# zhangyi-3/UCDIR

Measured on AMD Instinct MI355X. Metric: restored images/sec at 50-step p_sample_loop, 256x256 SID, higher is better.
Workload: dtype bf16

## Files before the change

### ucdir_amd/csrc/engine.hip

```cpp
#include <hip/hip_runtime.h>

#include <cmath>
#include <cstdio>
#include <cstring>
#include <map>
#include <mutex>
#include <set>
#include <array>
#include <atomic>
#include <memory>
#include <string>
#include <vector>

#include "../../include/ucdir_hip.h"
#include "cgemm.hip.h"
#include "conv_halo.hip.h"
#include "akgm_halo.hip.h"
#include "akgm_pre.hip.h"
#include "akgm_ws.hip.h"
#include "akgm_ws32.hip.h"
#include "akgm_ws64.hip.h"
#include "conv_ws.hip.h"
#include "conv_sk.hip.h"
#include "conv_ws128.hip.h"
// ... 714 lines not shown
        nblk *= p.usplit;
    }
    p.own_tc = !env().no_owntc && w.Tbb != nullptr;
    p.Tbb = w.Tbb; p.Tgt = w.Tg;

    AkgmKind kind = pre ? AkgmKind::PRE : (!env().no_attlds && (w.cg == 16 || w.cg == 32)) ? AkgmKind::HALO_ATTLDS : AkgmKind::HALO_STAGE;
    const bool use_ws = !env().no_ws;
    if (pre && use_ws && w.C == 64 && y.H % 16 == 0 && y.W % 16 == 0 && p.th == 16 && p.tw == 16 &&
        (g_persist_grid > 0 || (long long)y.B * p.tiles_x * p.tiles_y >= 4LL * num_cus()))
        kind = AkgmKind::WS;
    if (use_ws && !env().no_ws16 && w.Apre != nullptr && w.cg == 16 && w.C == 128 && y.H % 16 == 0 && y.W % 16 == 0 &&
        (g_persist_grid > 0 || (long long)y.B * (y.H / 16) * (y.W / 16) * 2 >= 4LL * num_cus()))
        kind = AkgmKind::WS16;
    int th32 = 0;
    for (int cand : {32, 24, 16, 8}) if (y.H % cand == 0) { th32 = cand; break; }
    const bool wsb_all = g_wsb > 0;
    const int nb32 = w.C / 32;
    if (use_ws && !env().no_ws32 && w.Aws32 != nullptr && (w.cg == 32 || (wsb_all && (w.cg == 16 || w.cg == 8))) && w.C == 8 * w.cg && th32 > 0 && y.W % 8 == 0 &&
        (g_persist_grid > 0 || (long long)y.B * (y.H / th32) * (y.W / 8) * nb32 >= 4LL * num_cus()))
        kind = AkgmKind::WS32;
    int tps64 = 0, grid64 = 0, hpos64 = 0;
    if (use_ws && !env().no_ws64 && w.Aws64 != nullptr && w.cg == 64 && w.C == 512 && y.H >= 2 && (y.H + 2) * (y.W + 2) < 32768) {
        const int nrole = 128 / AkWs64::NW;
        grid64 = num_cus() / nrole * nrole; if (grid64 < nrole) grid64 = nrole;
        const int span = (y.H - 1) * (y.W + 2) + y.W, nslots = grid64 / nrole;
        for (int cand : {4, 2}) {
            const int hpos = 32 * cand + 2 * (y.W + 2) + 2;
            if (hpos > AkWs64::HPOS) continue;
            const int tps = (span + 32 * cand - 1) / (32 * cand);
            const bool enough = cand == 4 ? (long long)y.B * tps >= 4LL * nslots : 2LL * y.B * span >= 3LL * nslots * hpos;
            if (g_persist_grid > 0 || enough) {
                kind = cand == 4 ? AkgmKind::WS64_4 : AkgmKind::WS64_2;
                tps64 = tps; hpos64 = hpos;
                break;
            }
        }
    }

    void (*kernel)(AkgmHP) = akgm_halo_stage_kernel;
    int key = KEY_AKGM_HALO, grid = nblk, threads = HC_THREADS, lds = AH_LDS;
    switch (kind) {
        case AkgmKind::WS64_4: case AkgmKind::WS64_2:
            p.A = w.Aws64; p.th = kind == AkgmKind::WS64_4 ? 4 : 2; p.tw = AkWs64::HBYTES(hpos64); p.tiles_x = tps64; p.tiles_y = 1;
            kernel = kind == AkgmKind::WS64_4 ? akgm_ws64_kernel<4, 8, true> : akgm_ws64_kernel<2, 8, true>;
            key = KEY_AKGM_WS64; grid = grid64; threads = 512; lds = AkWs64::lds(hpos64);
            break;
        case AkgmKind::WS32: {
            p.A = w.Aws32; p.th = th32; p.tw = 8; p.tiles_x = y.W / 8; p.tiles_y = y.H / th32;
            const int ntiles = y.B * p.tiles_x * p.tiles_y;
            int ncu = num_cus() / nb32 * nb32; if (ncu < nb32) ncu = nb32;
            grid = nb32 * ntiles < ncu ? nb32 * ntiles : ncu;
            kernel = w.cg == 32 ? akgm_ws32_kernel<32> : w.cg == 16 ? akgm_ws32_kernel<16> : akgm_ws32_kernel<8>;
            key = KEY_AKGM_WS32; lds = AkWs32::LDS;
            break;
        }
        case AkgmKind::WS: {
            const int ntiles = y.B * p.tiles_x * p.tiles_y, ncu = num_cus();
            grid = ntiles < ncu ? ntiles : ncu;
            kernel = akgm_ws_kernel<8>; key = KEY_AKGM_WS; lds = AkWs::LDS;
            break;
        }
        case AkgmKind::WS16: {
            p.A = w.Apre; p.th = 16; p.tw = 16; p.tiles_x = y.W / 16; p.tiles_y = y.H / 16;
            int ncu = num_cus() & ~1; if (ncu < 2) ncu = 2;
            const int ntiles = y.B * p.tiles_x * p.tiles_y;
            grid = 2 * ntiles < ncu ? 2 * ntiles : ncu;
            kernel = akgm_ws_kernel<16>; key = KEY_AKGM_WS16; lds = AkWs::LDS;
            break;
        }
        case AkgmKind::PRE: kernel = akgm_pre_kernel<8>; key = KEY_AKGM_PRE; lds = AkPre<8>::LDS; break;
        case AkgmKind::HALO_ATTLDS: kernel = akgm_halo_kernel<true>; break;
        case AkgmKind::HALO_STAGE: break;
    }
    if (!p.own_tc)
        hipLaunchKernelGGL(akgm_tc_kernel, dim3(9 * ((8 * w.C + 1023) / 1024), y.B), dim3(256), 0, st, h1.stats, inv_cnt, w.bias, w.Tb, w.Tg, 8 * w.C, tcbuf, msbuf);
    const ProfEntry e{key, 2.0 * 9 * w.C * (double)w.C * y.H * y.W * y.B, (3.0 * w.C * 2 + 32) * (double)y.H * y.W * y.B + 9.0 * w.C * w.C * 2, y.H, y.W, w.C, w.C};
    StampDump sd(st, STAMPS_256); p.dbg = sd.dbg();
    bracket(e, st, [&] { hipLaunchKernelGGL(kernel, dim3(grid), dim3(threads), lds, st, p); });
    sd.print([&](int, int n) { fprintf(stderr, "AKGM TIMING cg=%d n=%d:", w.cg, n); });
}

static void run_akgm(const AkgmW& w, const Act& h1, const float* G, const float* attw, const Act& res, Act& y,
                     float* tcbuf, hipStream_t st) {
    const int C = w.C;
    require(C == 64 || C % 128 == 0, "AKGM: channel count must be 64 or a multiple of 128");
    if (g_use_halo && (w.cg == 8 || w.cg == 16 || w.cg == 32 || w.cg == 64)) { run_akgm_halo(w, h1, G, attw, res, y, tcbuf, st); return; }
    require(w.Kpad != 640, "AKGM weights packed for the halo kernel");
    GemmP p; zero_gemm(p);
    const int TM = (C == 64) ? 64 : 128;
    p.A = w.A; p.a_ld = w.Kpad; p.a_rows = C; p.a_gstride = (long long)C * w.Kpad;
    p.B0 = h1.p; p.b0_bstride = h1.bstride(); p.ld0 = C; p.c0 = C;
    p.cols_mode = COLS_S1;
    p.H = y.H; p.W = y.W; p.Wp = y.W + 2; p.Hi = y.H; p.Wi = y.W; p.Wpi = p.Wp;
    p.p0 = p.Wp + 1; p.pn = (y.H - 1) * p.Wp + y.W;
    p.ntaps = 9; p.cg = w.cg; p.cpt = w.cg / 8; p.cpt_shift = ilog2(p.cpt);
    p.nk = w.Kpad / CG_BK;
    p.tiles = (p.pn + CG_TP - 1) / CG_TP;
    p.groups_per_wg = (C == 64) ? 8 : 1;
    p.rowtiles = (C == 64) ? 1 : 8 * (C / TM);
    p.nbatch = y.B;
    p.fold = 1; p.act = 1;
    p.stats0 = h1.stats; p.inv_count = 1.0 / ((double)C * h1.H * h1.W);
    p.bias = w.bias; p.Tb = w.Tb; p.Tg = w.Tg; p.tab_ld = 8 * C;
    p.res = res.p; p.res_bstride = res.bstride(); p.res_ld = res.C; p.res_coff = 0;
    p.out = y.p; p.out_bstride = y.bstride(); p.out_ld = C; p.nfeat = C;
    p.G = G; p.g_bstride = (long long)y.H * y.W * 8; p.attw = attw;
    p.stats_out = y.stats;
    launch_cgemm(p, TM, EPI_AKGM, st);
}

struct AttnBufs {
    bf16_t* qkv = nullptr;
    float* S = nullptr;
    bf16_t* P = nullptr;
    bf16_t* Vt = nullptr;
    int N = 0, Npad = 0, C = 0, B = 0;
    bool flash = true, half = false;
};

static std::atomic<int> g_flash{-1};
static bool flash_ok(int C) {
    const bool on = g_flash < 0 ? !env().no_flash : g_flash != 0;
    return on && C % 128 == 0 && C <= 512;
}

static void alloc_attn(DevPool& pool, AttnBufs& a, int B, int N, int C, bool half) {
    a.B = B; a.N = N; a.C = C; a.Npad = ((N + 63) / 64) * 64;
    a.half = half; a.flash = flash_ok(C);
    if (a.flash && !half && g_flash < 0 && B * ((N + FA_BQ - 1) / FA_BQ) < 32) a.flash = false;
    require(a.flash || !half, "fp16 attention operands need the flash kernel (C % 128 == 0, C <= 512)");
    a.qkv = (bf16_t*)pool.alloc((size_t)B * N * 3 * C * 2);
    if (!a.flash) {
        a.S = (float*)pool.alloc((size_t)B * N * a.Npad * 4);
        a.P = (bf16_t*)pool.alloc((size_t)B * N * a.Npad * 2);
    }
    a.Vt = (bf16_t*)pool.alloc((size_t)B * C * a.Npad * 2);
}

static std::vector<float> fold_out_into_v(const float* wqkv, const float* wout, int C) {
    std::vector<float> w(wqkv, wqkv + (size_t)3 * C * C);
    std::vector<double> row(C);
    for (int o = 0; o < C; ++o) {
        for (int i = 0; i < C; ++i) row[i] = 0.0;
        for (int m = 0; m < C; ++m) {
            const double a = wout[(size_t)o * C + m];
            const float* wv = wqkv + ((size_t)2 * C + m) * C;
            for (int i = 0; i < C; ++i) row[i] += a * (double)wv[i];
        }
        for (int i = 0; i < C; ++i) w[((size_t)2 * C + o) * C + i] = (float)row[i];
    }
    return w;
}

static void run_attention(const ConvW& wqkv, const ConvW& wout, const Act& x, Act& y, AttnBufs& a, hipStream_t st) {
    const int C = x.C, N = x.H * x.W, B = x.B, Npad = ((N + 63) / 64) * 64;
    require(C % 128 == 0, "attention: channels must be a multiple of 128");
    require((size_t)N <= (size_t)a.N && C == a.C && B <= a.B, "attention buffers too small");
    const bool qws = !env().no_qkv_ws && wqkv.Aqkv && !a.half && (C == 256 || C == 512);
    if (qws) {
        QkvP q;
        q.A = wqkv.Aqkv; q.x = x.p; q.x_bstride = x.bstride();
        q.H = x.H; q.W = x.W; q.Wp = x.W + 2; q.N = N; q.nbatch = B; q.tps = (N + 127) / 128; q.rowtiles = 3 * C / 256;
        q.stats = x.stats; q.inv_count = 1.0 / ((double)C * N);
        q.Tb = wqkv.Tb; q.Tg = wqkv.Tg;
        q.qkv = a.qkv; q.qkv_bstride = (long long)N * 3 * C; q.ld = 3 * C;
        q.vt = a.Vt; q.vt_bstride = (long long)C * Npad; q.Npad = Npad;
        const int units = q.rowtiles * B * q.tps, ncu = num_cus();
        const int grid = units < ncu ? units : ncu;
        const ProfEntry e{KEY_QKV_WS, 2.0 * 3 * C * (double)C * N * B, ((double)N * C * 2 + (double)N * 3 * C * 2) * B + 3.0 * C * C * 2, x.H, x.W, C, 3 * C};
        bracket(e, st, [&] {
            if (C == 512) hipLaunchKernelGGL(qkv_ws_kernel<512>, dim3(grid), dim3(HC_THREADS), QkvWs::LDS, st, q);
            else hipLaunchKernelGGL(qkv_ws_kernel<256>, dim3(grid), dim3(HC_THREADS), QkvWs::LDS, st, q);
        });
    } else {
    {
        GemmP p; zero_gemm(p);
        p.A = wqkv.A; p.a_ld = wqkv.Kpad; p.a_rows = wqkv.rows_pad;
        p.B0 = x.p; p.b0_bstride = x.bstride(); p.ld0 = C; p.c0 = C;
        p.cols_mode = COLS_S1; p.H = x.H; p.W = x.W; p.Wp = x.W + 2; p.Hi = x.H; p.Wi = x.W; p.Wpi = p.Wp;
        p.p0 = p.Wp + 1; p.pn = (x.H - 1) * p.Wp + x.W;
        p.ntaps = 1; p.cg = C; p.cpt = C / 8; p.nk = C / CG_BK;
        p.tiles = (p.pn + CG_TP - 1) / CG_TP; p.rowtiles = wqkv.rows_pad / 128; p.nbatch = B;
        p.fold = 1; p.stats0 = x.stats; p.inv_count = 1.0 / ((double)C * N);
        p.Tb = wqkv.Tb; p.Tg = wqkv.Tg; p.tab_ld = 3 * C; p.bias = nullptr;
        p.out = a.qkv; p.out_bstride = (long long)N * 3 * C; p.out_ld = 3 * C; p.out_compact = 1; p.nfeat = 3 * C;
        p.out_f16 = a.half ? 1 : 0;
        launch_cgemm(p, 128, EPI_STD, st);
    }
    hipLaunchKernelGGL(transpose_v_kernel, dim3((Npad + 31) / 32, C / 32, B), dim3(256), 0, st,
                       a.qkv, N, 3 * C, 2 * C, C, Npad, a.Vt);
    }
    if (a.flash) {
        FlashP f;
        f.qkv = a.qkv; f.qkv_bstride = (long long)N * 3 * C; f.ld = 3 * C;
        f.vt = a.Vt; f.vt_bstride = (long long)C * Npad; f.Npad = Npad;
        f.N = N; f.C = C; f.W = x.W;
        f.scale_log2e = 1.4426950408889634f / sqrtf((float)C);
        f.bias = wout.bias;
        f.res = x.p; f.res_bstride = x.bstride(); f.out = y.p; f.out_bstride = y.bstride();
        f.stats_out = y.stats;
        f.nq = (N + FA_BQ - 1) / FA_BQ;
        StampDump sd(st, STAMPS_256); f.dbg = sd.dbg();
        const dim3 grid((unsigned)(B * f.nq));
        const size_t lds = fa_lds_bytes(C);
        const ProfEntry e{a.half ? KEY_FLASH_F16 : KEY_FLASH, 4.0 * (double)N * N * C * B, ((double)N * 3 * C * 2 + 2.0 * N * C * 2) * B, x.H, x.W, C, C};
        bracket(e, st, [&] {
            switch (C / 128 * 2 + (a.half ? 1 : 0)) {
                case 2: hipLaunchKernelGGL((flash_attn2_kernel<1, false>), grid, dim3(FA_THREADS), lds, st, f); break;
                case 3: hipLaunchKernelGGL((flash_attn2_kernel<1, true>), grid, dim3(FA_THREADS), lds, st, f); break;
                case 4: hipLaunchKernelGGL((flash_attn2_kernel<2, false>), grid, dim3(FA_THREADS), lds, st, f); break;
                case 5: hipLaunchKernelGGL((flash_attn2_kernel<2, true>), grid, dim3(FA_THREADS), lds, st, f); break;
                case 6: hipLaunchKernelGGL((flash_attn2_kernel<3, false>), grid, dim3(FA_THREADS), lds, st, f); break;
                case 7: hipLaunchKernelGGL((flash_attn2_kernel<3, true>), grid, dim3(FA_THREADS), lds, st, f); break;
                case 8: hipLaunchKernelGGL((flash_attn2_kernel<4, false>), grid, dim3(FA_THREADS), lds, st, f); break;
                default: hipLaunchKernelGGL((flash_attn2_kernel<4, true>), grid, dim3(FA_THREADS), lds, st, f); break;
            }
        });
        sd.print([&](int, int n) { fprintf(stderr, "FLASH TIMING N=%d C=%d B=%d stamps=%d:", N, C, B, n); });
        return;
    }
    {
        GemmP p; zero_gemm(p);
        p.A = a.qkv + C; p.a_bstride = (long long)N * 3 * C; p.a_ld = 3 * C; p.a_rows = N;
        p.B0 = a.qkv; p.b0_bstride = (long long)N * 3 * C; p.ld0 = 3 * C; p.c0 = C;
        p.cols_mode = COLS_PLAIN; p.H = 1; p.W = N; p.Wp = N; p.p0 = 0; p.pn = N;
        p.ntaps = 1; p.cg = C; p.cpt = C / 8; p.nk = C / CG_BK;
        p.tiles = (N + CG_TP - 1) / CG_TP; p.rowtiles = (N + 127) / 128; p.nbatch = B;
        p.alpha = 1.0f / sqrtf((float)C);
        p.out = a.S; p.out_f32 = 1; p.out_bstride = (long long)N * Npad; p.out_ld = Npad; p.nfeat = N;
        launch_cgemm(p, 128, EPI_STD, st);
    }
    {
        const long long rows = (long long)B * N;
        const dim3 g((unsigned)((rows + 3) / 4));
        if (Npad <= 64 * 4 * 2) hipLaunchKernelGGL((softmax_kernel<2>), g, dim3(256), 0, st, a.S, a.P, rows, N, Npad);
        else if (Npad <= 64 * 4 * 6) hipLaunchKernelGGL((softmax_kernel<6>), g, dim3(256), 0, st, a.S, a.P, rows, N, Npad);
        else hipLaunchKernelGGL((softmax_kernel<0>), g, dim3(256), 0, st, a.S, a.P, rows, N, Npad);
    }
    {
        GemmP p; zero_gemm(p);
        p.A = a.Vt; p.a_bstride = (long long)C * Npad; p.a_ld = Npad; p.a_rows = C;
        p.B0 = a.P; p.b0_bstride = (long long)N * Npad; p.ld0 = Npad; p.c0 = Npad;
        p.cols_mode = COLS_PLAIN; p.H = 1; p.W = N; p.Wp = N; p.p0 = 0; p.pn = N;
        p.ntaps = 1; p.cg = Npad; p.cpt = Npad / 8; p.nk = Npad / CG_BK;
        p.tiles = (N + CG_TP - 1) / CG_TP; p.rowtiles = C / 128; p.nbatch = B;
        p.bias = wout.bias;
        p.plain_w = x.W;
        p.res = x.p; p.res_bstride = x.bstride(); p.res_ld = C;
        p.out = y.p; p.out_bstride = y.bstride(); p.out_ld = C; p.nfeat = C;
        p.stats_out = y.stats;
        launch_cgemm(p, 128, EPI_STD, st);
    }
    HIPC(hipGetLastError());
}

struct LayerDesc {
    std::string kind, name;
    int level = 0, cin = 0, cout = 0, skip_c = 0; bool attn = false, push_skip = false;
};

static std::vector<LayerDesc> build_layers(const ucdir_config& c) {
    std::vector<LayerDesc> L;
    const int inner = c.inner_channel, nm = c.n_mults;
    int pre = inner, res = c.image_size, level = 0, idx = 1;
    std::vector<int> feat{pre};
    auto in_attn = [&](int r) { for (int i = 0; i < c.n_attn_res; ++i) if (c.attn_res[i] == r) return true; return false; };
    { LayerDesc d; d.kind = "stem"; d.name = "downs.0"; d.cin = c.in_channel; d.cout = inner; d.push_skip = true; L.push_back(d); }
    for (int ind = 0; ind < nm; ++ind) {
        const bool last = ind == nm - 1, ua = in_attn(res);
        const int cm = inner * c.channel_mults[ind];
        for (int r = 0; r < c.res_blocks; ++r) {
            LayerDesc d; d.kind = "block"; d.name = "downs." + std::to_string(idx++); d.level = level;
            d.cin = pre; d.cout = cm; d.attn = ua; d.push_skip = true; L.push_back(d);
            feat.push_back(cm); pre = cm;
        }
        if (!last) {
            LayerDesc d; d.kind = "down"; d.name = "downs." + std::to_string(idx++); d.level = level;
            d.cin = pre; d.cout = pre; d.push_skip = true; L.push_back(d);
            feat.push_back(pre); res /= 2; ++level;
        }
    }
    { LayerDesc d; d.kind = "block"; d.name = "mid.0"; d.level = level; d.cin = pre; d.cout = pre; d.attn = true; L.push_back(d); }
    { LayerDesc d; d.kind = "block"; d.name = "mid.1"; d.level = level; d.cin = pre; d.cout = pre; L.push_back(d); }
    idx = 0;
    for (int ind = nm - 1; ind >= 0; --ind) {
        const bool last = ind < 1, ua = in_attn(res);
        const int cm = inner * c.channel_mults[ind];
        for (int r = 0; r < c.res_blocks + 1; ++r) {
            const int sc = feat.back(); feat.pop_back();
            LayerDesc d; d.kind = "block"; d.name = "ups." + std::to_string(idx++); d.level = level;
            d.cin = pre + sc; d.cout = cm; d.skip_c = sc; d.attn = ua; L.push_back(d);
            pre = cm;
        }
        if (!last) {
            LayerDesc d; d.kind = "up"; d.name = "ups." + std::to_string(idx++); d.level = level;
            d.cin = pre; d.cout = pre; L.push_back(d);
            res *= 2; --level;
        }
    }
    return L;
}

struct HostT { std::vector<float> v; std::vector<int64_t> shape; };

struct LayerW {
    ConvW conv;
    ConvW resconv; bool has_res = false;
    AkgmW sp;
    ConvW qkv, outp;
    float* gw = nullptr;
    bf16_t* stem_w = nullptr;
    int block_index = -1;
};

struct LayerRT {
    Act out;
    Act h1, res, bo;
    float* G = nullptr;
};

struct ucdir_ctx {
// ... 560 lines not shown
    const std::string w("ucdir_image_metrics");
    require(a && b && workspace && sse && ssim_sum, w + ": null argument");
    require(B > 0 && H > 0 && W > 0, w + ": bad shape");
    require(C == 1 || C == 3, w + ": C must be 1 or 3");
    require((int64_t)B * C <= 65535, w + ": more than 65535 (image, channel) pairs");
    require(((uintptr_t)workspace & 7) == 0 && ((uintptr_t)sse & 7) == 0 && ((uintptr_t)ssim_sum & 7) == 0,
            w + ": workspace and outputs must be 8-byte aligned");
    hipPointerAttribute_t pa;
    HIPC(hipPointerGetAttributes(&pa, a));
    require(pa.type == hipMemoryTypeDevice, w + ": a is not a device pointer");
    const void* others[4] = {b, workspace, sse, ssim_sum};
    const char* names[4] = {"b", "workspace", "sse", "ssim_sum"};
    for (int i = 0; i < 4; ++i) {
        hipPointerAttribute_t po;
        HIPC(hipPointerGetAttributes(&po, others[i]));
        require(po.type == hipMemoryTypeDevice && po.device == pa.device, w + ": " + names[i] + " must live on the device of a");
    }
    int nx, ny;
    image_metrics_grid(H, W, nx, ny);
    const long long ntiles = (long long)nx * ny;
    require(ntiles <= 0x7fffffffLL, w + ": image too large");
    ImageMetricsTaps taps;
    for (int k = 0; k < 11; ++k) taps.w[k] = std::exp(-(double)((k - 5) * (k - 5)) / (2 * 1.5 * 1.5));
    double tot = ((taps.w[0] + taps.w[1]) + (taps.w[2] + taps.w[3])) + ((taps.w[4] + taps.w[5]) + (taps.w[6] + taps.w[7]));
    tot += taps.w[8];
    tot += taps.w[9];
    tot += taps.w[10];
    for (int k = 0; k < 11; ++k) taps.w[k] /= tot;
    DevGuard dg(pa.device);
    double* part_ssim = (double*)workspace;
    unsigned long long* part_sse = (unsigned long long*)(part_ssim + (long long)B * C * ntiles);
    hipLaunchKernelGGL(image_metrics_tile_kernel, dim3((unsigned)ntiles, (unsigned)(B * C)), dim3(256), 0, (hipStream_t)stream,
                       a, (long long)a_sn, (long long)a_sc, (long long)a_sh, b, (long long)b_sn, (long long)b_sc, (long long)b_sh,
                       C, H, W, nx, ny, taps, part_ssim, part_sse);
    HIPC(hipGetLastError());
    hipLaunchKernelGGL(image_metrics_finish_kernel, dim3((unsigned)(B * C)), dim3(256), 0, (hipStream_t)stream, part_ssim, part_sse,
                       (int)ntiles, (int)(H > 10 && W > 10), (unsigned long long*)sse, ssim_sum);
    HIPC(hipGetLastError());
    API_END
}

int64_t ucdir_jpeg_roundtrip_workspace_bytes(int32_t B, int32_t H, int32_t W) {
    if (B <= 0 || H < 16 || W < 16) return -1;
    const int64_t H16 = (H + 15) & ~15, W16 = (W + 15) & ~15;
    return (int64_t)B * H16 * W16 * 3 / 2;
}

int32_t ucdir_jpeg_roundtrip(const uint8_t* in, uint8_t* out, int32_t B, int32_t H, int32_t W, int32_t quality, int32_t bgr,
                             void* workspace, void* stream) {
    API_BEGIN
    const std::string w("ucdir_jpeg_roundtrip");
    require(quality >= 1 && quality <= 100, w + ": quality must lie in 1..100");
    require(B > 0 && H >= 16 && W >= 16, w + ": bad shape (B > 0, H and W at least 16)");
    require((int64_t)B * H * W < (1LL << 31), w + ": more than 2^31 - 1 pixels");
    require(in && out && workspace, w + ": null argument");
    require(((uintptr_t)workspace & 7) == 0, w + ": workspace must be 8-byte aligned");
    hipPointerAttribute_t pa;
    HIPC(hipPointerGetAttributes(&pa, in));
    require(pa.type == hipMemoryTypeDevice, w + ": in is not a device pointer");
    const void* others[2] = {out, workspace};
    const char* names[2] = {"out", "workspace"};
    for (int i = 0; i < 2; ++i) {
        hipPointerAttribute_t po;
        HIPC(hipPointerGetAttributes(&po, others[i]));
        require(po.type == hipMemoryTypeDevice && po.device == pa.device, w + ": " + names[i] + " must live on the device of in");
    }
    static const int std_luma[64] = {16, 11, 10, 16, 24, 40, 51, 61, 12, 12, 14, 19, 26, 58, 60, 55, 14, 13, 16, 24, 40, 57, 69, 56,
                                     14, 17, 22, 29, 51, 87, 80, 62, 18, 22, 37, 56, 68, 109, 103, 77, 24, 35, 55, 64, 81, 104, 113, 92,
                                     49, 64, 78, 87, 103, 121, 120, 101, 72, 92, 95, 98, 112, 100, 103, 99};
    static const int std_chroma4[16] = {17, 18, 24, 47, 18, 21, 26, 66, 24, 26, 56, 99, 47, 66, 99, 99};
    const int scale = quality < 50 ? 5000 / quality : 200 - 2 * quality;
    JpegQuant qt;
    for (int i = 0; i < 64; ++i) {
        const int r = i >> 3, c = i & 7;
        const int sc = (r < 4 && c < 4) ? std_chroma4[r * 4 + c] : 99;
        qt.q[0][i] = std::min(std::max((std_luma[i] * scale + 50) / 100, 1), 255);
        qt.q[1][i] = std::min(std::max((sc * scale + 50) / 100, 1), 255);
    }
    DevGuard dg(pa.device);
    const long long nmcu = (long long)B * ((H + 15) / 16) * ((W + 15) / 16);
    hipLaunchKernelGGL(jpeg_mcu_kernel, dim3((unsigned)((nmcu + JPEG_MCUS_PER_WG - 1) / JPEG_MCUS_PER_WG)), dim3(256), 0,
                       (hipStream_t)stream, in, (unsigned char*)workspace, B, H, W, bgr ? 1 : 0, qt);
    HIPC(hipGetLastError());
    const long long npix = (long long)B * H * W;
    hipLaunchKernelGGL(jpeg_upsample_kernel, dim3((unsigned)((npix + 255) / 256)), dim3(256), 0, (hipStream_t)stream,
                       (const unsigned char*)workspace, out, B, H, W, bgr ? 1 : 0);
    HIPC(hipGetLastError());
    API_END
}

int32_t ucdir_set_graph(ucdir_ctx* ctx, int32_t on) {
    API_BEGIN
    require(ctx, "null ctx");
    DevGuard dg(ctx->cfg.device);
    ctx->use_graph = on != 0;
    if (!on) ctx->drop_graphs();
    API_END
}

int32_t ucdir_sampler_step(float* x_t, const float* eps, const float* noise, int64_t n, float c_recip, float c_recipm1,
                           float coef1, float coef2, float sigma, void* stream) {
    API_BEGIN
    require(x_t && eps, "null argument");
    hipPointerAttribute_t pa;
    HIPC(hipPointerGetAttributes(&pa, x_t));
    require(pa.type == hipMemoryTypeDevice, "ucdir_sampler_step: x_t is not a device pointer");
    DevGuard dg(pa.device);
    long long blocks = (n + 255) / 256; if (blocks > 4096) blocks = 4096;
    hipLaunchKernelGGL(sampler_step_kernel, dim3((unsigned)blocks), dim3(256), 0, (hipStream_t)stream, x_t, eps,
                       sigma != 0.f ? noise : nullptr, (long long)n, c_recip, c_recipm1, coef1, coef2, sigma);
    HIPC(hipGetLastError());
    API_END
}

int32_t ucdir_debug_read(ucdir_ctx* ctx, const char* layer, const char* what, float* dst, int64_t dst_elems, void* stream) {
    API_BEGIN
    require(ctx && layer && what && dst, "null argument");
    DevGuard dg(ctx->cfg.device);
    require(!ctx->acts_reused, "ucdir_debug_read: activation buffers of this (large) shape are recycled by lifetime; set "
                               "UCDIR_KEEP_ACTS=1 before planning to keep every layer's tensor");
    for (size_t li = 0; li < ctx->layers.size(); ++li) {
        if (ctx->layers[li].name != layer) continue;
        const LayerRT& r = ctx->rt[li];
        if (!strcmp(what, "attw")) {
            require(ctx->layers[li].kind == "block" && ctx->attw != nullptr, "attw: not a residual block");
            require(dst_elems == (int64_t)ctx->B * 8, "debug_read: attw has B * 8 elements");
            HIPC(hipMemcpyAsync(dst, ctx->attw + (size_t)ctx->lw[li].block_index * ctx->B * 8, sizeof(float) * ctx->B * 8,
                                hipMemcpyDeviceToDevice, (hipStream_t)stream));
            return 0;
        }
        const Act* a = &r.out;
        if (!strcmp(what, "h1")) a = &r.h1;
        else if (!strcmp(what, "res")) a = &r.res;
        else if (!strcmp(what, "bo")) a = &r.bo;
        require(a->p != nullptr, "no such activation");
        const int64_t n = (int64_t)a->B * a->C * a->H * a->W;
        require(n == dst_elems, "debug_read: dst has " + std::to_string(dst_elems) + " elements, activation has " + std::to_string(n));
        hipLaunchKernelGGL(act_to_nchw_kernel, dim3(2048), dim3(256), 0, (hipStream_t)stream, a->p, dst, a->B, a->C, a->H, a->W);
        HIPC(hipGetLastError());
        return 0;
    }
    throw std::runtime_error(std::string("unknown layer ") + layer);
    API_END
}

int32_t ucdir_debug_flag(const char* name, int32_t value) {
    API_BEGIN
    require(name != nullptr, "null argument");
    if (!strcmp(name, "flash")) g_flash = value;
    else if (!strcmp(name, "splitk")) g_splitk = value;
    else if (!strcmp(name, "wsb")) g_wsb = value;
    else if (!strcmp(name, "skmix")) g_skmix = value;
    else if (!strcmp(name, "convsk")) g_convsk = value;
    else if (!strcmp(name, "persist_grid")) g_persist_grid = value;
    else throw std::runtime_error(std::string("unknown debug flag ") + name);
    API_END
}

int32_t ucdir_debug_launch_plan(const char* what, int32_t wgs, int32_t nchunks, int32_t steps_per_chunk, double out_elems) {
    if (!what) return -1;
    try {
        if (!strcmp(what, "ksplit")) return choose_ksplit(wgs, nchunks, steps_per_chunk, out_elems);
        if (!strcmp(what, "usplit")) return choose_usplit(wgs);
    } catch (...) {}
    return -1;
}

int32_t ucdir_profile_enable(int32_t on) {
    API_BEGIN
    g_prof.on = on != 0;
    API_END
}

int32_t ucdir_profile_read(int32_t cap, int32_t* keys, int32_t* launches, double* ms, double* flops, double* bytes,
                           int32_t* nrows, void* stream) {
    API_BEGIN
    HIPC(hipStreamSynchronize((hipStream_t)stream));
    std::map<int, int> idx; int n = 0;
    const bool detail = env().prof_detail;
    struct Det { int n = 0; double ms = 0, flops = 0; };
    std::map<std::array<int, 5>, Det> det;
    for (auto& e : g_prof.entries) {
        float t = 0.f; HIPC(hipEventElapsedTime(&t, e.e0, e.e1));
        if (detail) { Det& d = det[{e.key, e.dH, e.dW, e.dCin, e.dCout}]; d.n++; d.ms += t; d.flops += e.flops; }
        auto it = idx.find(e.key);
        int r;
        if (it == idx.end()) { if (n >= cap) continue; r = n++; idx[e.key] = r; keys[r] = e.key; launches[r] = 0; ms[r] = 0; flops[r] = 0; bytes[r] = 0; }
        else r = it->second;
        launches[r] += 1; ms[r] += t; flops[r] += e.flops; bytes[r] += e.bytes;
    }
    *nrows = n;
    for (auto& kv : det)
        fprintf(stderr, "PROF key=%d H=%d W=%d cin=%d cout=%d launches=%d ms=%.4f TF=%.1f\n", kv.first[0], kv.first[1], kv.first[2],
                kv.first[3], kv.first[4], kv.second.n, kv.second.ms, kv.second.flops / (kv.second.ms * 1e9 + 1e-30));
    g_prof.entries.clear(); g_prof.used = 0;
    API_END
}

int32_t ucdir_matrix_rate(int32_t iters, int32_t random, double* tflops, void* stream) {
    API_BEGIN
    if (iters <= 0 || !tflops) throw std::runtime_error("ucdir_matrix_rate: iters > 0 and a result pointer are required");
    hipStream_t st = (hipStream_t)stream;
    struct Probe {
        float* sink = nullptr; hipEvent_t e0 = nullptr, e1 = nullptr;
        ~Probe() { if (e0) (void)hipEventDestroy(e0); if (e1) (void)hipEventDestroy(e1); if (sink) (void)hipFree(sink); }
    } pr;
    HIPC(hipMalloc((void**)&pr.sink, 4));
    HIPC(hipEventCreate(&pr.e0)); HIPC(hipEventCreate(&pr.e1));
    const int grid = 2 * num_cus();
    float best = 1e30f;
    for (int r = 0; r < 4; ++r) {
        HIPC(hipEventRecord(pr.e0, st));
        hipLaunchKernelGGL(matrix_rate_kernel, dim3(grid), dim3(256), 0, st, iters, random, pr.sink);
        HIPC(hipEventRecord(pr.e1, st)); HIPC(hipEventSynchronize(pr.e1));
        float ms = 0.f; HIPC(hipEventElapsedTime(&ms, pr.e0, pr.e1));
        if (r && ms < best) best = ms;
    }
    *tflops = 2.0 * 32 * 32 * 16 * 8.0 * iters * 4 * grid / (best * 1e-3) / 1e12;
    API_END
}

int64_t ucdir_workspace_bytes(const ucdir_ctx* ctx) { return ctx ? ctx->apool.bytes + ctx->wpool.bytes : 0; }
double ucdir_forward_flops(const ucdir_ctx* ctx) { return ctx ? ctx->flops : 0.0; }

static Act act_from_nchw(DevPool& pool, const float* x, int B, int C, int H, int W, hipStream_t st, bool stats) {
    Act a = make_act(pool, B, H, W, C, true);
    hipLaunchKernelGGL(nchw_to_act_kernel, dim3(2048), dim3(256), 0, st, x, a.p, B, C, H, W);
    if (stats) hipLaunchKernelGGL(act_stats_kernel, dim3(B), dim3(256), 0, st, a.p, H, W, C, a.stats);
    HIPC(hipGetLastError());
    return a;
}

static void read_stats(const Act& out, int B, double* stats_out_host, hipStream_t st) {
    std::vector<stat_t> sfx;
    if (stats_out_host) { sfx.resize((size_t)2 * UCDIR_STAT_SLOTS * B); HIPC(hipMemcpyAsync(sfx.data(), out.stats, sizeof(stat_t) * sfx.size(), hipMemcpyDeviceToHost, st)); }
    HIPC(hipStreamSynchronize(st));
    if (stats_out_host)
        for (int bb = 0; bb < B; ++bb)
            for (int q = 0; q < 2; ++q) {
                stat_t acc = 0;
                for (int k = 0; k < UCDIR_STAT_SLOTS; ++k) acc += sfx[((size_t)bb * UCDIR_STAT_SLOTS + k) * 2 + q];
                stats_out_host[bb * 2 + q] = (double)acc / UCDIR_STAT_SCALE;
            }
}

int32_t ucdir_op_conv(const float* x0, int32_t c0, const float* x1, int32_t c1, int32_t B, int32_t H, int32_t W,
                      const float* w_host, const float* bias_host, const float* gamma_host, const float* beta_host,
                      int32_t cout, int32_t ksize, int32_t mode, int32_t silu, const float* residual, float* y,
                      double* stats_out_host, void* stream) {
    API_BEGIN
    ensure_kernel_attrs();
    hipStream_t st = (hipStream_t)stream;
    DevPool pool;
    Act a0 = act_from_nchw(pool, x0, B, c0, H, W, st, true);
    Act a1; if (x1) a1 = act_from_nchw(pool, x1, B, c1, H, W, st, true);
    int Ho = H, Wo = W;
    if (mode == COLS_DOWN) { Ho = H / 2; Wo = W / 2; } else if (mode == COLS_UP) { Ho = 2 * H; Wo = 2 * W; }
    Act out = make_act(pool, B, Ho, Wo, cout);
    Act res; if (residual) res = act_from_nchw(pool, residual, B, cout, Ho, Wo, st, false);
    ConvW w = upload_conv(pool, w_host, bias_host, gamma_host, beta_host, cout, c0 + (x1 ? c1 : 0), ksize);
    if (mode == COLS_UP && ksize == 3) upload_upconv(pool, w, w_host, bias_host);
    run_conv(w, mode, {a0, x1 ? &a1 : nullptr, out, silu, residual ? &res : nullptr, true}, st);
    hipLaunchKernelGGL(act_to_nchw_kernel, dim3(2048), dim3(256), 0, st, out.p, y, B, cout, Ho, Wo);
    HIPC(hipGetLastError());
    read_stats(out, B, stats_out_host, st);
    API_END
}

int32_t ucdir_op_conv_res(const float* x0, int32_t c0, const float* x1, int32_t c1, int32_t B, int32_t H, int32_t W,
                          const float* w_host, const float* bias_host, const float* gamma_host, const float* beta_host,
                          const float* wres_host, const float* bres_host, int32_t cout, int32_t silu,
                          float* y, float* yres, double* stats_out_host, void* stream) {
    API_BEGIN
    ensure_kernel_attrs();
    hipStream_t st = (hipStream_t)stream;
    DevPool pool;
    const int cin = c0 + (x1 ? c1 : 0);
    Act a0 = act_from_nchw(pool, x0, B, c0, H, W, st, true);
    Act a1; if (x1) a1 = act_from_nchw(pool, x1, B, c1, H, W, st, true);
    Act out = make_act(pool, B, H, W, cout), rout = make_act(pool, B, H, W, cout, false);
    ConvW w = upload_conv(pool, w_host, bias_host, gamma_host, beta_host, cout, cin, 3);
    ConvW wr = upload_conv(pool, wres_host, bres_host, nullptr, nullptr, cout, cin, 1);
    if (w.TM == 64 && cin % 64 == 0 && w.Kpad == 9 * cin) {
        PackedConv P = pack_conv(w_host, nullptr, gamma_host, beta_host, cout, cin, 3, 64);
        const std::vector<bf16_t> a10 = pack_conv_res10(P, wres_host);
        w.A10 = pool.upload(a10); w.bias_res = wr.bias;
        if (cin == 128 && cout == 64) w.Aws128 = pool.upload(pack_conv_ws128(a10));
    }
    const bool did = run_conv(w, COLS_S1, {a0, x1 ? &a1 : nullptr, out, silu, nullptr, true, &rout, &wr}, st);
    if (!did) run_conv(wr, COLS_S1, {a0, x1 ? &a1 : nullptr, rout, 0, nullptr, false}, st);
    hipLaunchKernelGGL(act_to_nchw_kernel, dim3(2048), dim3(256), 0, st, out.p, y, B, cout, H, W);
    hipLaunchKernelGGL(act_to_nchw_kernel, dim3(2048), dim3(256), 0, st, rout.p, yres, B, cout, H, W);
    HIPC(hipGetLastError());
    read_stats(out, B, stats_out_host, st);
    API_END
}

int32_t ucdir_op_akgm(const float* h, const float* att, const float* res, int32_t B, int32_t C, int32_t H, int32_t W,
                      const float* wsp_host, const float* bsp_host, const float* gamma_host, const float* beta_host,
                      float* y, double* stats_out_host, void* stream) {
    API_BEGIN
    ensure_kernel_attrs();
    hipStream_t st = (hipStream_t)stream;
    DevPool pool;
    Act ah = act_from_nchw(pool, h, B, C, H, W, st, true);
    Act ar = act_from_nchw(pool, res, B, C, H, W, st, false);
    Act out = make_act(pool, B, H, W, C);
    float* G = (float*)pool.alloc((size_t)B * H * W * 8 * 4);
    hipLaunchKernelGGL(nchw8_to_compact_kernel, dim3(1024), dim3(256), 0, st, att, G, B, H, W);
    std::vector<float> ones((size_t)B * 8, 1.f);
    float* attw = pool.upload(ones);
    AkgmW w = upload_akgm(pool, wsp_host, bsp_host, gamma_host, beta_host, C);
    float* tcbuf = (float*)pool.alloc((size_t)B * (9 * 8 * C + 2) * sizeof(float), false);
    run_akgm(w, ah, G, attw, ar, out, tcbuf, st);
    hipLaunchKernelGGL(act_to_nchw_kernel, dim3(2048), dim3(256), 0, st, out.p, y, B, C, H, W);
    HIPC(hipGetLastError());
// ... 271 lines not shown
```

### ucdir_amd/csrc/qkv_ws.hip.h

```cpp
#pragma once
#include "akgm_ws.hip.h"

struct QkvP {
    const bf16_t* A;
    const bf16_t* x; long long x_bstride;
    int H, W, Wp, N, nbatch, tps, rowtiles;
    const stat_t* stats; double inv_count;
    const float* Tb; const float* Tg;
    bf16_t* qkv; long long qkv_bstride; int ld;
    bf16_t* vt; long long vt_bstride; int Npad;
};

struct QkvWs {
    static constexpr int CHUNK = 128 * 256;
    static constexpr int NBUF = 3;
    static constexpr int OFF_TBM = NBUF * CHUNK;
    static constexpr int OFF_SCAL = OFF_TBM + 1024;
    static constexpr int LDS = OFF_SCAL + 64;
};

template <int C>
__global__ __launch_bounds__(HC_THREADS, 2) void qkv_ws_kernel(const QkvP p) {
    constexpr int NKS = C / 16;
    constexpr int NCH = C / 128;
    extern __shared__ __attribute__((aligned(16))) unsigned char smem[];
    float* const tbm = reinterpret_cast<float*>(smem + QkvWs::OFF_TBM);
    float* const scal = reinterpret_cast<float*>(smem + QkvWs::OFF_SCAL);
    const int tid = threadIdx.x, lane = tid & 63, l31 = lane & 31, hh = lane >> 5;
    const int wave = __builtin_amdgcn_readfirstlane(tid >> 6);
    int lid;
    {
        const int nblk = gridDim.x, bid = blockIdx.x;
        const int q = nblk >> 3, r = nblk & 7, xcd = bid & 7;
        lid = (xcd < r ? xcd * (q + 1) : r * (q + 1) + (xcd - r) * q) + (bid >> 3);
    }
    const int RT = p.rowtiles, rt = lid % RT, slot = lid / RT;
    const int nwg = ((int)gridDim.x - rt + RT - 1) / RT;
    const int T = p.nbatch * p.tps;
    const int t_beg = (int)((long long)slot * T / nwg), t_end = (int)((long long)(slot + 1) * T / nwg);
    if (t_beg >= t_end) return;
    const bool is_v = rt * 256 >= 2 * C;

    bf16x8_t af[NKS];
    {
        const unsigned char* Ab = reinterpret_cast<const unsigned char*>(p.A) + ((long long)(rt * 8 + wave) * NKS) * 1024 + lane * 16;
#pragma unroll
        for (int j = 0; j < NKS; ++j) af[j] = *reinterpret_cast<const bf16x8_t*>(Ab + j * 1024);
    }
#pragma unroll
    for (int j = 0; j < NKS; ++j) asm volatile("" : "+v"(af[j]));

    const int pxl = is_v ? (16 * ((l31 >> 2) & 1) + 4 * (l31 >> 3) + (l31 & 3)) : l31;
    auto swz = [](int px) { return px & 15; };
    const unsigned fr0 = pxl * 256 + ((hh ^ swz(pxl)) << 4);

    int b_cur = -1;
    float rstd = 1.f;
    unsigned prel[4];
    auto tile_prel = [&](int tn) {
#pragma unroll
        for (int i = 0; i < 4; ++i) {
            const int px = 4 * (8 * i + wave) + (lane >> 4);
            int n = tn * 128 + px; n = n < p.N ? n : p.N - 1;
            const int y = n / p.W, x = n - y * p.W;
            prel[i] = (unsigned)(((y + 1) * p.Wp + x + 1) * C + (((lane & 15) ^ swz(px)) << 3)) * 2;
        }
    };
    auto issue_chunk = [&](int tb, int c, int buf) {
        const unsigned char* xb = reinterpret_cast<const unsigned char*>(p.x + (long long)tb * p.x_bstride) + c * 256;
#pragma unroll
        for (int i = 0; i < 4; ++i)
            __builtin_amdgcn_global_load_lds((const GLOBAL_AS void*)(xb + prel[i]), (LDS_AS void*)(smem + buf * QkvWs::CHUNK + (8 * i + wave) * 1024), 16, 0, 0);
    };

    int tb = t_beg / p.tps, tn = t_beg - tb * p.tps;
    int it = t_beg, ib = tb, in = tn, ic = 0, ibuf = 0, ahead = 0;
    tile_prel(in);
    auto issue_next = [&]() {
        if (it >= t_end) return;
        issue_chunk(ib, ic, ibuf);
        ibuf = ibuf + 1 == QkvWs::NBUF ? 0 : ibuf + 1;
        ++ahead;
        if (++ic == NCH) {
            ic = 0; ++it;
            if (++in == p.tps) { in = 0; ++ib; }
            if (it < t_end) tile_prel(in);
        }
    };
    issue_next();
    issue_next();
    int gbuf = 0;

    auto tile_loop = [&](auto vtag) {
    constexpr bool VT = decltype(vtag)::value;
#pragma unroll 1
    for (int t = t_beg; t < t_end; ++t) {
        int nb = tb, nn = tn + 1;
        if (nn == p.tps) { nn = 0; ++nb; }
        if (tb != b_cur) {
            asm volatile("s_barrier" ::: "memory");
            b_cur = tb;
            if (tid == 0) {
                double S, Q; float mean, r2;
                stat_read(p.stats, nullptr, tb, S, Q);
                mean_rstd(S, Q, p.inv_count, mean, r2);
                scal[0] = mean * r2; scal[1] = r2;
            }
            asm volatile("s_waitcnt lgkmcnt(0)\n\ts_barrier" ::: "memory");
            rstd = scal[1];
            if (tid < 256) tbm[tid] = p.Tb[rt * 256 + tid] - scal[0] * p.Tg[rt * 256 + tid];
        }
        f32x16_t acc[4];
#pragma unroll
        for (int tp = 0; tp < 4; ++tp)
#pragma unroll
            for (int e = 0; e < 16; ++e) acc[tp][e] = 0.f;

#pragma unroll
        for (int c = 0; c < NCH; ++c) {
            if (ahead >= 2) asm volatile("s_waitcnt vmcnt(4) lgkmcnt(0)\n\ts_barrier" ::: "memory");
            else asm volatile("s_waitcnt vmcnt(0) lgkmcnt(0)\n\ts_barrier" ::: "memory");
            --ahead;
            issue_next();
            const unsigned bb = gbuf * QkvWs::CHUNK;
            bf16x8_t xf[3][2];
            auto frag = [&](auto sc, bf16x8_t (&dst)[2]) {
                constexpr int st = decltype(sc)::value, j = st >> 1, th = st & 1;
                const unsigned fa = bb + (fr0 ^ (32u * j));
                lds_read16_asm<(2 * th) * 8192>(dst[0], fa);
                lds_read16_asm<(2 * th + 1) * 8192>(dst[1], fa);
            };
            __builtin_amdgcn_sched_barrier(0);
            frag(std::integral_constant<int, 0>{}, xf[0]);
            frag(std::integral_constant<int, 1>{}, xf[1]);
            __builtin_amdgcn_s_setprio(1);
            static_for<0, 16>([&](auto sc) {
                constexpr int st = decltype(sc)::value, j = st >> 1, th = st & 1;
                if constexpr (st + 2 < 16) frag(std::integral_constant<int, st + 2>{}, xf[(st + 2) % 3]);
                constexpr int younger = (st + 2 < 16) ? 4 : ((st + 1 < 16) ? 2 : 0);
                lgkm_wait_asm<younger>();
#pragma unroll
                for (int tq = 0; tq < 2; ++tq)
                    acc[2 * th + tq] = VT ? __builtin_amdgcn_mfma_f32_32x32x16_bf16(xf[st % 3][tq], af[8 * c + j], acc[2 * th + tq], 0, 0, 0)
                                          : __builtin_amdgcn_mfma_f32_32x32x16_bf16(af[8 * c + j], xf[st % 3][tq], acc[2 * th + tq], 0, 0, 0);
            });
            __builtin_amdgcn_s_setprio(0);
            gbuf = gbuf + 1 == QkvWs::NBUF ? 0 : gbuf + 1;
        }

        const int n0 = tn * 128;
        if constexpr (!VT) {
            const int f0 = 32 * wave + 16 * hh;
            bf16_t* ob = p.qkv + (long long)tb * p.qkv_bstride + rt * 256 + f0;
#pragma unroll
            for (int tp = 0; tp < 4; ++tp) {
                const int n = n0 + 32 * tp + l31;
                bf16_t* op = ob + (long long)n * p.ld;
#pragma unroll
                for (int h8 = 0; h8 < 2; ++h8) {
                    const f32x4_t c0 = *reinterpret_cast<const f32x4_t*>(smem + QkvWs::OFF_TBM + (f0 + 8 * h8) * 4);
                    const f32x4_t c1 = *reinterpret_cast<const f32x4_t*>(smem + QkvWs::OFF_TBM + (f0 + 8 * h8 + 4) * 4);
                    float v[8];
#pragma unroll
                    for (int e = 0; e < 4; ++e) { v[e] = fmaf(acc[tp][8 * h8 + e], rstd, c0[e]); v[4 + e] = fmaf(acc[tp][8 * h8 + 4 + e], rstd, c1[e]); }
                    if (n < p.N) *reinterpret_cast<uint4*>(op + 8 * h8) = pack8_bf16(v);
                }
            }
        } else {
            const int f = 32 * wave + l31;
            const float cst = tbm[f];
            bf16_t* ob = p.vt + (long long)tb * p.vt_bstride + (long long)(rt * 256 - 2 * C + f) * p.Npad;
#pragma unroll
            for (int tp = 0; tp < 4; ++tp) {
                const int n = n0 + 32 * tp + 16 * hh;
#pragma unroll
                for (int h8 = 0; h8 < 2; ++h8) {
                    float v[8];
#pragma unroll
                    for (int e = 0; e < 8; ++e) v[e] = fmaf(acc[tp][8 * h8 + e], rstd, cst);
                    if (n < p.Npad) *reinterpret_cast<uint4*>(ob + n + 8 * h8) = pack8_bf16(v);
                }
            }
        }
        tb = nb; tn = nn;
    }
    };
    if (is_v) tile_loop(std::true_type{}); else tile_loop(std::false_type{});
}
```

Before: 37.18.

## Flatten QKV tile indexing across batch boundaries to avoid padded partial tiles

Enumerates the QKV projection's 128-pixel tiles over the concatenated batch*N pixel range instead of padding each image to a multiple of 128. Tiles that straddle an image boundary now hold per-image normalization constants in double-buffered LDS slots and route output rows to the right batch. The A-fragment register load is moved after the first prefetches so it overlaps them. This removes wasted MMA work on padded tail tiles when N is not a multiple of 128, at the cost of more index arithmetic, extra V-transpose pad filling, and more complex epilogue branches.

Result: no change. 37.10, median of 2 (-0.2%).

```diff
diff --git a/ucdir_amd/csrc/engine.hip b/ucdir_amd/csrc/engine.hip
--- a/ucdir_amd/csrc/engine.hip
+++ b/ucdir_amd/csrc/engine.hip
@@ -890,6 +890,42 @@
     return w;
 }
 
+static std::atomic<int> g_qkvflat{-1};
+static bool qkv_want_flat() { return g_qkvflat != 0; }
+static int qkv_grid(int wgs, int rowtiles, int T) {
+    const long long units = (long long)rowtiles * T;
+    const int g = units < wgs ? (int)units : wgs;
+    return g < rowtiles ? rowtiles : g;
+}
+static int qkv_plan_query(bool miscovered, int wgs, int B, int N, int rowtiles) {
+    require(wgs > 0 && B > 0 && N > 0 && rowtiles > 0, "qkv plan: bad arguments");
+    int flat, T, wrap;
+    qkv_ws_tiles(qkv_want_flat(), B, N, flat, T, wrap);
+    const int grid = qkv_grid(wgs, rowtiles, T);
+    std::vector<int> cover(miscovered ? (size_t)rowtiles * B * N : 0, 0);
+    int worst = 0;
+    for (int lid = 0; lid < grid; ++lid) {
+        int rt, t0, t1;
+        qkv_ws_range(lid, grid, rowtiles, T, rt, t0, t1);
+        if (t1 - t0 > worst) worst = t1 - t0;
+        if (!miscovered) continue;
+        int b0 = (int)((long long)t0 * 128 / wrap), nA = (int)((long long)t0 * 128 - (long long)b0 * wrap);
+        for (int t = t0; t < t1; ++t) {
+            for (int i = 0; i < 128; ++i) {
+                int b = b0, n = nA + i;
+                if (n >= N) { if (flat && b0 + 1 < B) { b = b0 + 1; n -= N; } else continue; }
+                cover[((size_t)rt * B + b) * N + n] += 1;
+            }
+            nA += 128;
+            if (nA >= wrap) { nA -= wrap; ++b0; }
+        }
+    }
+    if (!miscovered) return worst;
+    int bad = 0;
+    for (int c : cover) bad += c != 1;
+    return bad;
+}
+
 static void run_attention(const ConvW& wqkv, const ConvW& wout, const Act& x, Act& y, AttnBufs& a, hipStream_t st) {
     const int C = x.C, N = x.H * x.W, B = x.B, Npad = ((N + 63) / 64) * 64;
     require(C % 128 == 0, "attention: channels must be a multiple of 128");
@@ -898,13 +934,13 @@
     if (qws) {
         QkvP q;
         q.A = wqkv.Aqkv; q.x = x.p; q.x_bstride = x.bstride();
-        q.H = x.H; q.W = x.W; q.Wp = x.W + 2; q.N = N; q.nbatch = B; q.tps = (N + 127) / 128; q.rowtiles = 3 * C / 256;
+        q.H = x.H; q.W = x.W; q.Wp = x.W + 2; q.N = N; q.nbatch = B; q.rowtiles = 3 * C / 256;
+        qkv_ws_tiles(qkv_want_flat() && 4 * x.bstride() < (1LL << 32), B, N, q.flat, q.T, q.wrap);
         q.stats = x.stats; q.inv_count = 1.0 / ((double)C * N);
         q.Tb = wqkv.Tb; q.Tg = wqkv.Tg;
         q.qkv = a.qkv; q.qkv_bstride = (long long)N * 3 * C; q.ld = 3 * C;
         q.vt = a.Vt; q.vt_bstride = (long long)C * Npad; q.Npad = Npad;
-        const int units = q.rowtiles * B * q.tps, ncu = num_cus();
-        const int grid = units < ncu ? units : ncu;
+        const int grid = qkv_grid(num_cus(), q.rowtiles, q.T);
         const ProfEntry e{KEY_QKV_WS, 2.0 * 3 * C * (double)C * N * B, ((double)N * C * 2 + (double)N * 3 * C * 2) * B + 3.0 * C * C * 2, x.H, x.W, C, 3 * C};
         bracket(e, st, [&] {
             if (C == 512) hipLaunchKernelGGL(qkv_ws_kernel<512>, dim3(grid), dim3(HC_THREADS), QkvWs::LDS, st, q);
@@ -1771,6 +1807,7 @@
     else if (!strcmp(name, "wsb")) g_wsb = value;
     else if (!strcmp(name, "skmix")) g_skmix = value;
     else if (!strcmp(name, "convsk")) g_convsk = value;
+    else if (!strcmp(name, "qkvflat")) g_qkvflat = value;
     else if (!strcmp(name, "persist_grid")) g_persist_grid = value;
     else throw std::runtime_error(std::string("unknown debug flag ") + name);
     API_END
@@ -1781,6 +1818,8 @@
     try {
         if (!strcmp(what, "ksplit")) return choose_ksplit(wgs, nchunks, steps_per_chunk, out_elems);
         if (!strcmp(what, "usplit")) return choose_usplit(wgs);
+        if (!strcmp(what, "qkv_max_tiles")) return qkv_plan_query(false, wgs, nchunks, steps_per_chunk, (int)out_elems);
+        if (!strcmp(what, "qkv_miscovered")) return qkv_plan_query(true, wgs, nchunks, steps_per_chunk, (int)out_elems);
     } catch (...) {}
     return -1;
 }
diff --git a/ucdir_amd/csrc/qkv_ws.hip.h b/ucdir_amd/csrc/qkv_ws.hip.h
--- a/ucdir_amd/csrc/qkv_ws.hip.h
+++ b/ucdir_amd/csrc/qkv_ws.hip.h
@@ -4,7 +4,8 @@
 struct QkvP {
     const bf16_t* A;
     const bf16_t* x; long long x_bstride;
-    int H, W, Wp, N, nbatch, tps, rowtiles;
+    int H, W, Wp, N, nbatch, rowtiles;
+    int flat, T, wrap;
     const stat_t* stats; double inv_count;
     const float* Tb; const float* Tg;
     bf16_t* qkv; long long qkv_bstride; int ld;
@@ -15,9 +16,22 @@
     static constexpr int CHUNK = 128 * 256;
     static constexpr int NBUF = 3;
     static constexpr int OFF_TBM = NBUF * CHUNK;
-    static constexpr int OFF_SCAL = OFF_TBM + 1024;
+    static constexpr int OFF_SCAL = OFF_TBM + 2048;
     static constexpr int LDS = OFF_SCAL + 64;
 };
+
+__host__ __device__ inline void qkv_ws_tiles(int want_flat, int nbatch, int N, int& flat, int& T, int& wrap) {
+    flat = (want_flat && N % 4 == 0 && N >= 128) ? 1 : 0;
+    const int tps = (N + 127) / 128;
+    T = flat ? (int)(((long long)nbatch * N + 127) / 128) : nbatch * tps;
+    wrap = flat ? N : tps * 128;
+}
+__host__ __device__ inline void qkv_ws_range(int lid, int nblk, int RT, int T, int& rt, int& t_beg, int& t_end) {
+    rt = lid % RT;
+    const int slot = lid / RT;
+    const int nwg = (nblk - rt + RT - 1) / RT;
+    t_beg = (int)((long long)slot * T / nwg); t_end = (int)((long long)(slot + 1) * T / nwg);
+}
 
 template <int C>
 __global__ __launch_bounds__(HC_THREADS, 2) void qkv_ws_kernel(const QkvP p) {
@@ -34,48 +48,42 @@
         const int q = nblk >> 3, r = nblk & 7, xcd = bid & 7;
         lid = (xcd < r ? xcd * (q + 1) : r * (q + 1) + (xcd - r) * q) + (bid >> 3);
     }
-    const int RT = p.rowtiles, rt = lid % RT, slot = lid / RT;
-    const int nwg = ((int)gridDim.x - rt + RT - 1) / RT;
-    const int T = p.nbatch * p.tps;
-    const int t_beg = (int)((long long)slot * T / nwg), t_end = (int)((long long)(slot + 1) * T / nwg);
+    int rt, t_beg, t_end;
+    qkv_ws_range(lid, (int)gridDim.x, p.rowtiles, p.T, rt, t_beg, t_end);
     if (t_beg >= t_end) return;
     const bool is_v = rt * 256 >= 2 * C;
-
-    bf16x8_t af[NKS];
-    {
-        const unsigned char* Ab = reinterpret_cast<const unsigned char*>(p.A) + ((long long)(rt * 8 + wave) * NKS) * 1024 + lane * 16;
-#pragma unroll
-        for (int j = 0; j < NKS; ++j) af[j] = *reinterpret_cast<const bf16x8_t*>(Ab + j * 1024);
-    }
-#pragma unroll
-    for (int j = 0; j < NKS; ++j) asm volatile("" : "+v"(af[j]));
 
     const int pxl = is_v ? (16 * ((l31 >> 2) & 1) + 4 * (l31 >> 3) + (l31 & 3)) : l31;
     auto swz = [](int px) { return px & 15; };
     const unsigned fr0 = pxl * 256 + ((hh ^ swz(pxl)) << 4);
 
-    int b_cur = -1;
-    float rstd = 1.f;
+    auto spans = [&](int b0) { return p.flat && b0 + 1 < p.nbatch; };
     unsigned prel[4];
-    auto tile_prel = [&](int tn) {
+    const unsigned xbs2 = (unsigned)(p.x_bstride * 2);
+    auto tile_prel = [&](int b0, int nA) {
+        int ot = tid; asm volatile("" : "+v"(ot));
+        const int px0 = 4 * wave + ((ot & 63) >> 4);
+        const unsigned swzb = (unsigned)(((ot & 15) ^ swz(px0)) << 4);
+        const bool two = spans(b0);
 #pragma unroll
         for (int i = 0; i < 4; ++i) {
-            const int px = 4 * (8 * i + wave) + (lane >> 4);
-            int n = tn * 128 + px; n = n < p.N ? n : p.N - 1;
-            const int y = n / p.W, x = n - y * p.W;
-            prel[i] = (unsigned)(((y + 1) * p.Wp + x + 1) * C + (((lane & 15) ^ swz(px)) << 3)) * 2;
-        }
-    };
-    auto issue_chunk = [&](int tb, int c, int buf) {
-        const unsigned char* xb = reinterpret_cast<const unsigned char*>(p.x + (long long)tb * p.x_bstride) + c * 256;
+            int n = nA + 32 * i + px0;
+            const bool over = n >= p.N;
+            n = over ? (two ? n - p.N : p.N - 1) : n;
+            const unsigned y = (unsigned)n / (unsigned)p.W, x = (unsigned)n - y * (unsigned)p.W;
+            prel[i] = ((y + 1) * (unsigned)p.Wp + x + 1) * (unsigned)(C * 2) + swzb + ((over && two) ? xbs2 : 0u);
+        }
+    };
+    auto issue_chunk = [&](int b0, int c, int buf) {
+        const unsigned char* xb = reinterpret_cast<const unsigned char*>(p.x + (long long)b0 * p.x_bstride) + c * 256;
 #pragma unroll
         for (int i = 0; i < 4; ++i)
             __builtin_amdgcn_global_load_lds((const GLOBAL_AS void*)(xb + prel[i]), (LDS_AS void*)(smem + buf * QkvWs::CHUNK + (8 * i + wave) * 1024), 16, 0, 0);
     };
 
-    int tb = t_beg / p.tps, tn = t_beg - tb * p.tps;
-    int it = t_beg, ib = tb, in = tn, ic = 0, ibuf = 0, ahead = 0;
-    tile_prel(in);
+    int tb = (int)((long long)t_beg * 128 / p.wrap), nA = (int)((long long)t_beg * 128 - (long long)tb * p.wrap);
+    int it = t_beg, ib = tb, inA = nA, ic = 0, ibuf = 0, ahead = 0;
+    tile_prel(ib, inA);
     auto issue_next = [&]() {
         if (it >= t_end) return;
         issue_chunk(ib, ic, ibuf);
@@ -83,32 +91,49 @@
         ++ahead;
         if (++ic == NCH) {
             ic = 0; ++it;
-            if (++in == p.tps) { in = 0; ++ib; }
-            if (it < t_end) tile_prel(in);
+            inA += 128;
+            if (inA >= p.wrap) { inA -= p.wrap; ++ib; }
+            if (it < t_end) tile_prel(ib, inA);
         }
     };
     issue_next();
     issue_next();
+
+    bf16x8_t af[NKS];
+    {
+        const unsigned char* Ab = reinterpret_cast<const unsigned char*>(p.A) + ((long long)(rt * 8 + wave) * NKS) * 1024 + lane * 16;
+#pragma unroll
+        for (int j = 0; j < NKS; ++j) af[j] = *reinterpret_cast<const bf16x8_t*>(Ab + j * 1024);
+    }
+#pragma unroll
+    for (int j = 0; j < NKS; ++j) asm volatile("" : "+v"(af[j]));
+
+    int cs_e = -1, cs_o = -1;
     int gbuf = 0;
 
     auto tile_loop = [&](auto vtag) {
     constexpr bool VT = decltype(vtag)::value;
 #pragma unroll 1
     for (int t = t_beg; t < t_end; ++t) {
-        int nb = tb, nn = tn + 1;
-        if (nn == p.tps) { nn = 0; ++nb; }
-        if (tb != b_cur) {
+        const bool two = spans(tb);
+        const int bl = (two && nA + 127 >= p.N) ? tb + 1 : tb;
+        if (((tb & 1) ? cs_o : cs_e) != tb || ((bl & 1) ? cs_o : cs_e) != bl) {
             asm volatile("s_barrier" ::: "memory");
-            b_cur = tb;
-            if (tid == 0) {
+            if (tid == 0 || (tid == 64 && bl != tb)) {
+                const int sb = tid == 0 ? tb : bl;
                 double S, Q; float mean, r2;
-                stat_read(p.stats, nullptr, tb, S, Q);
+                stat_read(p.stats, nullptr, sb, S, Q);
                 mean_rstd(S, Q, p.inv_count, mean, r2);
-                scal[0] = mean * r2; scal[1] = r2;
+                scal[2 * (sb & 1)] = mean * r2; scal[2 * (sb & 1) + 1] = r2;
             }
             asm volatile("s_waitcnt lgkmcnt(0)\n\ts_barrier" ::: "memory");
-            rstd = scal[1];
-            if (tid < 256) tbm[tid] = p.Tb[rt * 256 + tid] - scal[0] * p.Tg[rt * 256 + tid];
+            {
+                int ot = tid; asm volatile("" : "+v"(ot));
+                const int sb = ot < 256 ? tb : bl, f = ot & 255;
+                if (ot < 256 || bl != tb) tbm[256 * (sb & 1) + f] = p.Tb[rt * 256 + f] - scal[2 * (sb & 1)] * p.Tg[rt * 256 + f];
+            }
+            if (tb & 1) cs_o = tb; else cs_e = tb;
+            if (bl & 1) cs_o = bl; else cs_e = bl;
         }
         f32x16_t acc[4];
 #pragma unroll
@@ -148,41 +173,82 @@
             gbuf = gbuf + 1 == QkvWs::NBUF ? 0 : gbuf + 1;
         }
 
-        const int n0 = tn * 128;
+        int ot = tid; asm volatile("" : "+v"(ot));
+        const int l31 = ot & 31, hh = (ot >> 5) & 1;
+        const int sl0 = tb & 1, sl1 = sl0 ^ 1;
+        const float rs0 = scal[2 * sl0 + 1], rs1 = scal[2 * sl1 + 1];
         if constexpr (!VT) {
             const int f0 = 32 * wave + 16 * hh;
             bf16_t* ob = p.qkv + (long long)tb * p.qkv_bstride + rt * 256 + f0;
 #pragma unroll
             for (int tp = 0; tp < 4; ++tp) {
-                const int n = n0 + 32 * tp + l31;
-                bf16_t* op = ob + (long long)n * p.ld;
+                int n = nA + 32 * tp + l31;
+                const bool over = n >= p.N, nxt = over && two;
+                n = nxt ? n - p.N : n;
+                const float rstd = nxt ? rs1 : rs0;
+                const unsigned tab = QkvWs::OFF_TBM + (nxt ? sl1 : sl0) * 1024 + f0 * 4;
+                bf16_t* op = ob + (nxt ? p.qkv_bstride : 0) + (long long)n * p.ld;
 #pragma unroll
                 for (int h8 = 0; h8 < 2; ++h8) {
-                    const f32x4_t c0 = *reinterpret_cast<const f32x4_t*>(smem + QkvWs::OFF_TBM + (f0 + 8 * h8) * 4);
-                    const f32x4_t c1 = *reinterpret_cast<const f32x4_t*>(smem + QkvWs::OFF_TBM + (f0 + 8 * h8 + 4) * 4);
+                    const f32x4_t c0 = *reinterpret_cast<const f32x4_t*>(smem + tab + (8 * h8) * 4);
+                    const f32x4_t c1 = *reinterpret_cast<const f32x4_t*>(smem + tab + (8 * h8 + 4) * 4);
                     float v[8];
 #pragma unroll
                     for (int e = 0; e < 4; ++e) { v[e] = fmaf(acc[tp][8 * h8 + e], rstd, c0[e]); v[4 + e] = fmaf(acc[tp][8 * h8 + 4 + e], rstd, c1[e]); }
-                    if (n < p.N) *reinterpret_cast<uint4*>(op + 8 * h8) = pack8_bf16(v);
+                    if (!over || nxt) *reinterpret_cast<uint4*>(op + 8 * h8) = pack8_bf16(v);
                 }
             }
         } else {
             const int f = 32 * wave + l31;
-            const float cst = tbm[f];
+            const float cs0 = tbm[256 * sl0 + f], cs1 = tbm[256 * sl1 + f];
             bf16_t* ob = p.vt + (long long)tb * p.vt_bstride + (long long)(rt * 256 - 2 * C + f) * p.Npad;
-#pragma unroll
-            for (int tp = 0; tp < 4; ++tp) {
-                const int n = n0 + 32 * tp + 16 * hh;
-#pragma unroll
-                for (int h8 = 0; h8 < 2; ++h8) {
-                    float v[8];
-#pragma unroll
-                    for (int e = 0; e < 8; ++e) v[e] = fmaf(acc[tp][8 * h8 + e], rstd, cst);
-                    if (n < p.Npad) *reinterpret_cast<uint4*>(ob + n + 8 * h8) = pack8_bf16(v);
+            const int dl = (p.flat && nA + 128 >= p.N) ? p.N - 1 - nA - 16 * hh : -1;
+            const bool owner = dl >= 0 && (dl & 16) == 0;
+            unsigned padb = 0;
+            if (!p.flat || (p.N & 15) == 0) {
+#pragma unroll
+                for (int tp = 0; tp < 4; ++tp) {
+                    int n = nA + 32 * tp + 16 * hh;
+                    const bool nxt = n >= p.N && two;
+                    const bool ok = p.flat ? (n < p.N || nxt) : n < p.Npad;
+                    n = nxt ? n - p.N : n;
+                    const float rstd = nxt ? rs1 : rs0, cst = nxt ? cs1 : cs0;
+                    bf16_t* og = ob + (nxt ? p.vt_bstride : 0) + n;
+#pragma unroll
+                    for (int h8 = 0; h8 < 2; ++h8) {
+                        float v[8];
+#pragma unroll
+                        for (int e = 0; e < 8; ++e) v[e] = fmaf(acc[tp][8 * h8 + e], rstd, cst);
+                        const uint4 pk = pack8_bf16(v);
+                        if (ok) *reinterpret_cast<uint4*>(og + 8 * h8) = pk;
+                        padb = dl == 32 * tp + 8 * h8 + 3 ? pk.y : (dl == 32 * tp + 8 * h8 + 7 ? pk.w : padb);
+                    }
                 }
-            }
-        }
-        tb = nb; tn = nn;
+            } else {
+#pragma unroll
+                for (int tp = 0; tp < 4; ++tp) {
+#pragma unroll
+                    for (int q4 = 0; q4 < 4; ++q4) {
+                        int n = nA + 32 * tp + 16 * hh + 4 * q4;
+                        const bool over = n >= p.N, nxt = over && two;
+                        n = nxt ? n - p.N : n;
+                        const float rstd = nxt ? rs1 : rs0, cst = nxt ? cs1 : cs0;
+                        float v[4];
+#pragma unroll
+                        for (int e = 0; e < 4; ++e) v[e] = fmaf(acc[tp][4 * q4 + e], rstd, cst);
+                        const uint2 pk = make_uint2(pack2_bf16(v[0], v[1]), pack2_bf16(v[2], v[3]));
+                        if (!over || nxt) *reinterpret_cast<uint2*>(ob + (nxt ? p.vt_bstride : 0) + n) = pk;
+                        padb = dl == 32 * tp + 4 * q4 + 3 ? pk.y : padb;
+                    }
+                }
+            }
+            if (owner) {
+                const unsigned pp = (padb >> 16) * 0x10001u;
+                for (int n = p.N; n < p.Npad; n += 4) *reinterpret_cast<uint2*>(ob + n) = make_uint2(pp, pp);
+            }
+        }
+        nA += 128;
+        if (nA >= p.wrap) { nA -= p.wrap; ++tb; }
     }
     };
     if (is_v) tile_loop(std::true_type{}); else tile_loop(std::false_type{});
```
